# mgp25/OpenLTE

Measured on AMD Instinct MI355X. Metric: DL subframes/sec @20MHz 100RB 64QAM, full chain FFT->CE->demap->rate-unmatch->turbo(REF)->CRC (SURVEY 8d W4), higher is better.
Workload: dtype i8 IQ in, f32 FFT/CE/equaliser, i8 soft bits, i16 path metrics (differences exact modulo 2^16); 1 GPU; W4 full DL chain: 20 MHz/100 RB/64QAM, 9 allocations per subframe (8x12 PRB TBS 3240 + 1x4 PRB TBS 1064), 65536 subframes per GPU, int8 IQ in HBM; subframes_per_gpu=65536, N_ant=1, CFI=2, channel_estimate_form=compact, decoder=REF (reference-faithful, bit-exact), unique_subframes=96, streams_per_gpu=1

## Files before the change

openlte_amd/csrc/turbo.hip:

```cpp
#include <algorithm>
#include <cstring>
#include <initializer_list>
#include <type_traits>
#include <vector>

#include "plan_core.hpp"
#include "turbo_swar.h"

using namespace turbo_geom;

namespace {

constexpr uint32_t RX_NULL_AS_INT = 10000;


__device__ __forceinline__ int sbyte(uint32_t w, int k) { return (int)__builtin_amdgcn_sbfe(w, 8 * k, 8); }

typedef __attribute__((address_space(3))) const uint8_t  lds_u8_t;
typedef __attribute__((address_space(3))) const int8_t   lds_i8_t;
typedef __attribute__((address_space(3))) const uint16_t lds_u16_t;
__device__ __forceinline__ uint32_t lds_u8(uint32_t addr) { return *(lds_u8_t *)(uintptr_t)addr; }
__device__ __forceinline__ int      lds_i8(uint32_t addr) { return *(lds_i8_t *)(uintptr_t)addr; }
__device__ __forceinline__ uint32_t lds_u16(uint32_t addr) { return *(lds_u16_t *)(uintptr_t)addr; }

// ... 593 lines not shown
            uint32_t o[4];
#pragma unroll
            for (int j = 0; j < 4; j++)
                o[j] = pack4u(lds_u8(PREP_QTAB_AT + QTAB_HALF + v[Src::kPacked ? 0 : x][4 * j]), lds_u8(PREP_QTAB_AT + QTAB_HALF + v[Src::kPacked ? 0 : x][4 * j + 1]), lds_u8(PREP_QTAB_AT + QTAB_HALF + v[Src::kPacked ? 0 : x][4 * j + 2]), lds_u8(PREP_QTAB_AT + QTAB_HALF + v[Src::kPacked ? 0 : x][4 * j + 3]));
            Q[x] = make_uint4(o[0], o[1], o[2], o[3]);
        } else {
            int q[16];
            if (use_qtab) {
#pragma unroll
                for (int k = 0; k < 16; k++) {
                    const float f = v[Src::kPacked ? 0 : x][k];
                    const int   t = qtab[(int)fabsf(f)];
                    q[k]          = f < 0.0f ? -t : t;
                }
            } else {
#pragma unroll
                for (int k = 0; k < 16; k++) q[k] = (int)((float)v[Src::kPacked ? 0 : x][k] * 127.0f / mx);
            }
            Q[x] = pack16(q);
        }
        if (nv >= 0) *reinterpret_cast<uint4 *>(out.arr[x] + unit_off(tile_off, lane, u)) = Q[x];
    }
    if (nv >= 0) *reinterpret_cast<uint4 *>(q0_lds + 16 * u) = Q[0];
    __syncthreads();

    uint4 I0 = make_uint4(0, 0, 0, 0);
    if (nv > 0) {
        uint32_t idx[16];
        if constexpr (MULTI)
            load_idx16_at(reinterpret_cast<const_u32x4_t *>(reinterpret_cast<uintptr_t>(pi + 16 * (size_t)u)), nv, idx, K);
        else
            load_idx16(pi, u, nv, idx, K);
        I0 = gather16_bytes(PREP_Q0_AT, idx);
    }
    if (nv >= 0) *reinterpret_cast<uint4 *>(out.arr[3] + unit_off(tile_off, lane, u)) = I0;
    if (identity && src.hard_inputs()) {
        auto cnt4 = [](uint32_t a, uint32_t b) { return (a & 0x01010101u) + (b & 0x01010101u); };
        const uint32_t c1[4] = {cnt4(Q[1].x, Q[0].x), cnt4(Q[1].y, Q[0].y), cnt4(Q[1].z, Q[0].z), cnt4(Q[1].w, Q[0].w)};
        const uint32_t c2[4] = {cnt4(Q[2].x, I0.x), cnt4(Q[2].y, I0.y), cnt4(Q[2].z, I0.z), cnt4(Q[2].w, I0.w)};
        const uint32_t o1 = c1[0] | c1[1] | c1[2] | c1[3], o2 = c2[0] | c2[1] | c2[2] | c2[3];
        int w1max = (o1 & 0x02020202u) ? 254 : (o1 ? 127 : 0), w2max = (o2 & 0x02020202u) ? 254 : (o2 ? 127 : 0);
        block_max_i2(w1max, w2max, red_i);
        if (w1max != 0 && w2max != 0) {
            auto mag4 = [](uint32_t cnt, int W) { return W == 254 ? (cnt << 6) - ((cnt | (cnt >> 1)) & 0x01010101u) : (cnt << 7) - cnt; };
            if (nv >= 0) {
                *reinterpret_cast<uint4 *>(out.arr[4] + unit_off(tile_off, lane, u)) = make_uint4(mag4(c1[0], w1max), mag4(c1[1], w1max), mag4(c1[2], w1max), mag4(c1[3], w1max));
                *reinterpret_cast<uint4 *>(out.arr[5] + unit_off(tile_off, lane, u)) = make_uint4(mag4(c2[0], w2max), mag4(c2[1], w2max), mag4(c2[2], w2max), mag4(c2[3], w2max));
            }
            return;
        }
    }
    uint32_t w1[16], w2[16], w1m = 0, w2m = 0;
    abs_sum16(Q[1], Q[0], w1, w1m);
    abs_sum16(Q[2], I0, w2, w2m);
    int w1max = (int)w1m, w2max = (int)w2m;
    block_max_i2(w1max, w2max, red_i);
    auto closed = [](int W) { return W == 254 || W == 127; };
    auto closed16 = [](const uint32_t (&w)[16], int W) {
        uint32_t o[4];
#pragma unroll
        for (int j = 0; j < 4; j++) {
            const uint32_t p = pack4u(w[4 * j], w[4 * j + 1], w[4 * j + 2], w[4 * j + 3]);
            o[j] = W == 254 ? (p >> 1) & 0x7F7F7F7Fu : p;
        }
        return make_uint4(o[0], o[1], o[2], o[3]);
    };
    if (!(closed(w1max) && closed(w2max))) {
        const float W1 = (float)w1max, W2 = (float)w2max;
        for (uint32_t t = threadIdx.x; t < MTAB_N; t += blockDim.x) {
            const float w = (float)t;
            mtab1[t] = (int8_t)(int)(127.0f * (w / W1));
            mtab2[t] = (int8_t)(int)(127.0f * (w / W2));
        }
        __syncthreads();
    }
    if (nv >= 0) {
        *reinterpret_cast<uint4 *>(out.arr[4] + unit_off(tile_off, lane, u)) = closed(w1max) ? closed16(w1, w1max) : lookup16(0, w1);
        *reinterpret_cast<uint4 *>(out.arr[5] + unit_off(tile_off, lane, u)) = closed(w2max) ? closed16(w2, w2max) : lookup16(MTAB_N, w2);
    }
}


struct SisoPass {
    const uint8_t *in_a;
    const uint8_t *in_b;
    uint32_t      *sgn;
    uint32_t      *dec;
};
struct SisoArgs { SisoPass p[2]; };

typedef unsigned short v2u __attribute__((ext_vector_type(2)));
__device__ __forceinline__ uint32_t sign_bits(v2s n) { return __builtin_bit_cast(uint32_t, __builtin_bit_cast(v2u, n) >> 15); }

template <int S> __device__ __forceinline__ void acs_step2(v2s (&pm)[8], v2s x2, v2s y2, uint32_t &acc)
{
    const v2s mx = as_v2s(neg_mask(x2 ^ y2)), nmx = ~mx;
    const v2s uP = (x2 + y2) & nmx;
    const v2s uQ = (x2 - y2) & mx;
    const uint32_t m0p = neg_mask(x2) & 0xFFF8FFF8u;
    const v2s P2 = as_v2s(__builtin_amdgcn_bitop3_b32(as_u32(mx), m0p, 0xFFFCFFFCu, 0x06));
    const v2s Q2 = as_v2s(__builtin_amdgcn_bitop3_b32(as_u32(mx), m0p, 0xFFFCFFFCu, 0x60));
    const v2s n0 = pm[1] - pm[0], n1 = pm[3] - pm[2], n2 = pm[5] - pm[4], n3 = pm[7] - pm[6];
    constexpr uint32_t top = 0x00010001u << (15 - 4 * S);
    acc = __builtin_amdgcn_bitop3_b32(acc, neg_mask(n0), top, 0xF8);
    acc = __builtin_amdgcn_bitop3_b32(acc, neg_mask(n1), top >> 1, 0xF8);
    acc = __builtin_amdgcn_bitop3_b32(acc, neg_mask(n2), top >> 2, 0xF8);
    acc = __builtin_amdgcn_bitop3_b32(acc, neg_mask(n3), top >> 3, 0xF8);
    auto sel = [](v2s d, v2s yes, v2s no) { return bit_select(neg_mask(d), yes, no); };
    v2s nw[8];
    nw[0] = sel(n0 - P2, pm[1] + uP, pm[0] - uP);
    nw[4] = sel(n0 + P2, pm[1] - uP, pm[0] + uP);
    nw[1] = sel(n1 - Q2, pm[3] + uQ, pm[2] - uQ);
    nw[5] = sel(n1 + Q2, pm[3] - uQ, pm[2] + uQ);
    nw[2] = sel(n2 + Q2, pm[5] - uQ, pm[4] + uQ);
    nw[6] = sel(n2 - Q2, pm[5] + uQ, pm[4] - uQ);
    nw[3] = sel(n3 + P2, pm[7] - uP, pm[6] + uP);
    nw[7] = sel(n3 - P2, pm[7] + uP, pm[6] - uP);
#pragma unroll
    for (int s = 0; s < 8; s++) pm[s] = nw[s];
}

template <int R> __device__ __forceinline__ v2s byte_pair2(uint32_t w0, uint32_t w1)
{
    return as_v2s(__builtin_amdgcn_perm(w1, w0, (uint32_t)(4 + R) << 24 | 0x0C0000u | (uint32_t)R << 8 | 0x0Cu)) >> 7;
}


#ifndef SISO_WPE
#define SISO_WPE 4
#endif
template <bool MULTI, int MODE>
__global__ __launch_bounds__(256) __attribute__((amdgpu_waves_per_eu(SISO_WPE, 8))) void k_turbo_siso(SisoArgs args, uint32_t K_arg, uint32_t n_tiles_arg, MultiArgs ma,
                                                                                                         const uint32_t *__restrict__ order)
{
    constexpr uint32_t mode = MODE;
    constexpr int      NA = MODE ? 1 : 2;
    __shared__ uint32_t tb_lut[2048];
    for (uint32_t i = threadIdx.x; i < 2048; i += blockDim.x) tb_lut[i] = turbo_swar::traceback_entry(i >> 3, i & 7u);
    __syncthreads();
    const uint32_t lane = threadIdx.x & 63u;
    uint32_t       K = K_arg, n_tiles = n_tiles_arg, wv = blockIdx.x * 4 + (threadIdx.x >> 6), n_wv = mode ? n_tiles : (n_tiles + 1) / 2;
    size_t         seg_off = 0;
    if constexpr (MULTI) {
        if (order) wv = __builtin_amdgcn_readfirstlane(order[wv]);
        if (wv >= n_tiles_arg) return;
        const_seg_t &sg = multi_seg(ma, wv);
        K = sg.K; n_tiles = sg.n_tiles; seg_off = sg.arr_off;
        wv -= mode ? sg.wv23 : sg.wv1;
        n_wv = mode ? n_tiles : (n_tiles + 1) / 2;
    }
    const uint32_t Kp = kpad64(K), nblk = Kp >> 6;
    if (wv >= n_wv) return;
    const uint8_t *pa[2], *pb[2];
    uint32_t      *dec[2], *sgn[2];
#pragma unroll
    for (int h = 0; h < 2; h++) {
        const SisoPass &ps   = args.p[mode ? h : 0];
        const uint32_t  tile = mode ? wv : min(2 * wv + h, n_tiles - 1);
        const size_t    off  = seg_off + (size_t)tile * Kp * 64 + lane * 64;
        pa[h] = ps.in_a + off; pb[h] = ps.in_b + off;
        dec[h] = ps.dec + (seg_off >> 3) + ((size_t)tile * nblk * 64 + lane) * 8;
        sgn[h] = ps.sgn + (seg_off >> 5) + ((size_t)tile * nblk * 64 + lane) * 2;
    }

    v2s pm[8];
#pragma unroll
    for (int s = 0; s < 8; s++) pm[s] = (v2s)(0);

    uint4 A[NA][4], B[2][4];
#pragma unroll
    for (int h = 0; h < 2; h++)
#pragma unroll
        for (int q = 0; q < 4; q++) {
            if (h < NA) A[h][q] = reinterpret_cast<const uint4 *>(pa[h])[q];
            B[h][q] = reinterpret_cast<const uint4 *>(pb[h])[q];
        }
    for (uint32_t blk = 0; blk < nblk; blk++) {
        const uint32_t nxt = (blk + 1 < nblk) ? blk + 1 : blk;
        uint32_t       dw[2][8];
#pragma unroll
        for (int q = 0; q < 4; q++) {
#pragma unroll
            for (int g2 = 0; g2 < 2; g2++) {
                const int g = 2 * q + g2;
                uint32_t  acc_lo = 0, acc_hi = 0;
                if (blk * 64 + g * 8 < K) {
                    const uint32_t a0l = g2 ? A[0][q].z : A[0][q].x, a0h = g2 ? A[0][q].w : A[0][q].y;
                    const uint32_t a1l = g2 ? A[NA - 1][q].z : A[NA - 1][q].x, a1h = g2 ? A[NA - 1][q].w : A[NA - 1][q].y;
                    const uint32_t b0l = g2 ? B[0][q].z : B[0][q].x, b0h = g2 ? B[0][q].w : B[0][q].y;
                    const uint32_t b1l = g2 ? B[1][q].z : B[1][q].x, b1h = g2 ? B[1][q].w : B[1][q].y;
                    acs_step2<0>(pm, byte_pair2<0>(a0l, a1l), byte_pair2<0>(b0l, b1l), acc_lo);
                    acs_step2<1>(pm, byte_pair2<1>(a0l, a1l), byte_pair2<1>(b0l, b1l), acc_lo);
                    acs_step2<2>(pm, byte_pair2<2>(a0l, a1l), byte_pair2<2>(b0l, b1l), acc_lo);
                    acs_step2<3>(pm, byte_pair2<3>(a0l, a1l), byte_pair2<3>(b0l, b1l), acc_lo);
                    acs_step2<0>(pm, byte_pair2<0>(a0h, a1h), byte_pair2<0>(b0h, b1h), acc_hi);
                    acs_step2<1>(pm, byte_pair2<1>(a0h, a1h), byte_pair2<1>(b0h, b1h), acc_hi);
                    acs_step2<2>(pm, byte_pair2<2>(a0h, a1h), byte_pair2<2>(b0h, b1h), acc_hi);
                    acs_step2<3>(pm, byte_pair2<3>(a0h, a1h), byte_pair2<3>(b0h, b1h), acc_hi);
                }
                dw[0][g] = __builtin_amdgcn_perm(acc_lo, acc_hi, 0x05040100u);
                dw[1][g] = __builtin_amdgcn_perm(acc_lo, acc_hi, 0x07060302u);
            }
            if (q >= 2) {
#pragma unroll
                for (int qq = (q == 2 ? 0 : 3); qq <= (q == 2 ? 2 : 3); qq++)
#pragma unroll
                    for (int h = 0; h < 2; h++) {
                        if (h < NA) A[h][qq] = reinterpret_cast<const uint4 *>(pa[h] + (size_t)nxt * 4096)[qq];
                        B[h][qq] = reinterpret_cast<const uint4 *>(pb[h] + (size_t)nxt * 4096)[qq];
                    }
            }
        }
#pragma unroll
        for (int h = 0; h < 2; h++) {
            uint4 *dp = reinterpret_cast<uint4 *>(dec[h] + (size_t)blk * 64 * 8);
            dp[0] = make_uint4(dw[h][0], dw[h][1], dw[h][2], dw[h][3]);
            dp[1] = make_uint4(dw[h][4], dw[h][5], dw[h][6], dw[h][7]);
        }
    }

    int cur[2] = {0, 0};
    {
        int best[2] = {0, 0};
#pragma unroll
        for (int s = 1; s < 8; s++) {
            const uint32_t d  = as_u32(pm[s] - pm[0]);
            const int      dh[2] = {(int)__builtin_amdgcn_sbfe(d, 0, 16), (int)d >> 16};
#pragma unroll
            for (int h = 0; h < 2; h++)
                if (dh[h] < best[h]) { best[h] = dh[h]; cur[h] = s; }
        }
    }

    uint4 D[2][2], Dn[2][2];
#pragma unroll
    for (int h = 0; h < 2; h++) {
        const uint4 *dp = reinterpret_cast<const uint4 *>(dec[h] + (size_t)(nblk - 1) * 64 * 8);
        D[h][0] = dp[0];
        D[h][1] = dp[1];
    }
    for (int blk = (int)nblk - 1; blk >= 0; blk--) {
        const int prv = blk > 0 ? blk - 1 : 0;
#pragma unroll
        for (int h = 0; h < 2; h++) {
            const uint4 *dpn = reinterpret_cast<const uint4 *>(dec[h] + (size_t)prv * 64 * 8);
            Dn[h][0] = dpn[0];
            Dn[h][1] = dpn[1];
        }
        uint32_t sbits[2][2];
#pragma unroll
        for (int g = 7; g >= 0; g--) {
            if ((g & 3) == 3) sbits[0][g >> 2] = sbits[1][g >> 2] = 0;
            if ((uint32_t)blk * 64 + g * 8 < K) {
                uint32_t word[2];
#pragma unroll
                for (int h = 0; h < 2; h++) {
                    const uint4 dq = D[h][g >> 2];
                    word[h] = (g & 3) == 0 ? dq.x : (g & 3) == 1 ? dq.y : (g & 3) == 2 ? dq.z : dq.w;
                }
#pragma unroll
                for (int b = 0; b < 4; b++) {
#pragma unroll
                    for (int h = 0; h < 2; h++) {
                        const uint32_t e = tb_lut[((word[h] >> (8 * b)) & 0xFFu) << 3 | (uint32_t)cur[h]];
                        cur[h]           = (int)(e & 7u);
                        sbits[h][g >> 2]   = __builtin_amdgcn_alignbit(sbits[h][g >> 2], e, 30);
                    }
                }
            }
        }
#pragma unroll
        for (int h = 0; h < 2; h++) {
            *reinterpret_cast<uint2 *>(sgn[h] + (size_t)blk * 64 * 2) = make_uint2(sbits[h][0], sbits[h][1]);
            D[h][0] = Dn[h][0];
            D[h][1] = Dn[h][1];
        }
    }
}

struct SmallPar { uint32_t cw, uw; };

__device__ __forceinline__ uint2 map_compose(uint2 F, uint2 G)
{
    return make_uint2(__builtin_amdgcn_perm(F.y, F.x, G.x), __builtin_amdgcn_perm(F.y, F.x, G.y));
}
__device__ __forceinline__ uint32_t map_at(uint2 F, uint32_t s) { return ((s & 4u ? F.y : F.x) >> (8 * (s & 3u))) & 7u; }
template <int N> __device__ __forceinline__ uint2 map_row_shl(uint2 v, uint2 keep)
{
    return make_uint2((uint32_t)__builtin_amdgcn_update_dpp((int)keep.x, (int)v.x, 0x100 + N, 0xF, 0xF, false),
                      (uint32_t)__builtin_amdgcn_update_dpp((int)keep.y, (int)v.y, 0x100 + N, 0xF, 0xF, false));
}

template <bool MULTI>
__global__ __launch_bounds__(64) void k_turbo_siso_small(SisoArgs args, uint32_t K_arg, uint32_t n_cb_arg, uint32_t mode, uint32_t gpw, MultiArgs ma)
{
    extern __shared__ __attribute__((aligned(16))) uint32_t sm_small[];
    SmallPar (*par)[64][4] = reinterpret_cast<SmallPar(*)[64][4]>(sm_small);
    uint32_t K = K_arg, n_cb = n_cb_arg, bidx = blockIdx.x;
    size_t   seg_off = 0;
    if constexpr (MULTI) {
        const_seg_t &sg = multi_seg(ma, blockIdx.x);
        K = sg.K; n_cb = sg.n_cb; seg_off = sg.arr_off; bidx = blockIdx.x - (mode ? sg.ws23 : sg.ws1);
    }
    const uint32_t Kp = kpad64(K), n_w32 = Kp >> 5;
    uint32_t      *decw = sm_small + gpw * 64 * 4 * 2;
    const uint32_t lane = threadIdx.x, gi = lane >> 2, j = lane & 3u;
    const uint32_t T0 = bidx * gpw, n_tr = n_cb * (mode ? 2u : 1u);
    const uint32_t n_g = min(gpw, n_tr - T0);
    auto pass_of = [&](uint32_t g) -> const SisoPass & { return args.p[mode ? (T0 + g) & 1u : 0u]; };
    auto off_of  = [&](uint32_t g) -> size_t {
        const uint32_t cb = mode ? (T0 + g) >> 1 : T0 + g;
        return seg_off + (size_t)(cb >> 6) * Kp * 64 + (cb & 63u) * 64;
    };
    const uint32_t n_chunk = (K + 63) >> 6;

    uint32_t XY = 0;
    uint32_t accv = 0;
    const uint32_t half_sel = j < 2 ? 0x01000100u : 0x03020302u;
#ifdef SMALL_PAD
    uint32_t padv[4] = {lane, lane + 1, lane + 2, lane + 3};
#endif
    int xs[SMALL_G], ys[SMALL_G];
    auto fetch = [&](uint32_t ch) {
#pragma unroll
        for (uint32_t g = 0; g < SMALL_G; g++)
            if (g < n_g) {
                const size_t e = off_of(g) + (size_t)ch * 4096 + lane;
                xs[g] = (int8_t)pass_of(g).in_a[e];
                ys[g] = (int8_t)pass_of(g).in_b[e];
            }
    };
    fetch(0);
    for (uint32_t ch = 0; ch < n_chunk; ch++) {
#pragma unroll
        for (uint32_t g = 0; g < SMALL_G; g++) {
            if (g >= n_g) break;
            const int      x  = xs[g], y = ys[g];
            const int      m0 = x >> 31, mx = m0 ^ (y >> 31), nmx = ~mx;
            const int      uP = ((x + y) << 1) & nmx, uQ = ((x - y) << 1) & mx;
            const int      c4 = (m0 & 8) - 4, P2 = c4 & nmx, Q2 = c4 & mx;
            auto pm16 = [](int v) { return ((uint32_t)v & 0xFFFFu) | ((uint32_t)(-v) << 16); };
            const uint32_t cP = pm16(P2), uPw = pm16(uP), cQ = pm16(Q2), uQw = pm16(uQ);
            auto swp = [](uint32_t w) { return (w >> 16) | (w << 16); };
            uint4 *dst = reinterpret_cast<uint4 *>(&par[g][lane][0]);
            dst[0] = make_uint4(cP, uPw, cQ, uQw);
            dst[1] = make_uint4(swp(cQ), swp(uQw), swp(cP), swp(uPw));
        }
        __syncthreads();
        if (ch + 1 < n_chunk) fetch(ch + 1);
        const uint32_t n_t = min(64u, K - ch * 64);
        if (gi < n_g) {
            auto steps8 = [&](uint32_t t8) {
                SmallPar pr[8];
#pragma unroll
                for (int k = 0; k < 8; k++) pr[k] = par[gi][t8 + k][j];
#pragma unroll
                for (int k = 0; k < 8; k++) {
                    const uint32_t t0 = (uint32_t)__builtin_amdgcn_mov_dpp((int)XY, 0x88, 0xF, 0xF, false);
                    const uint32_t t1 = (uint32_t)__builtin_amdgcn_mov_dpp((int)XY, 0xDD, 0xF, 0xF, false);
                    const v2s a = as_v2s(__builtin_amdgcn_perm(t0, t0, half_sel)), b = as_v2s(__builtin_amdgcn_perm(t1, t1, half_sel));
                    const v2s n = b - a;
                    accv = __builtin_amdgcn_alignbit(accv, as_u32(n), 31);
                    const v2s uw = as_v2s(pr[k].uw);
                    XY = as_u32(bit_select(neg_mask(n - as_v2s(pr[k].cw)), b + uw, a - uw));
#ifdef SMALL_PAD
#pragma unroll
                    for (int z = 0; z < SMALL_PAD; z++) asm volatile("v_add_u32 %0, %0, %1" : "+v"(padv[z & 3]) : "v"(lane));
#endif
                }
            };
            uint32_t t = 0;
            for (; t + 32 <= n_t; t += 32) {
                steps8(t); steps8(t + 8); steps8(t + 16); steps8(t + 24);
                decw[(gi * n_w32 + ((ch * 64 + t) >> 5)) * 4 + j] = accv;
            }
            if (t < n_t) {
                const uint32_t w = (ch * 64 + t) >> 5, left = n_t - t;
                for (; t < n_t; t += 8) steps8(t);
                decw[(gi * n_w32 + w) * 4 + j] = accv << (32u - left);
            }
        }
        __syncthreads();
    }

#ifdef SMALL_PAD
    if ((padv[0] ^ padv[1] ^ padv[2] ^ padv[3]) == 0x12345678u) decw[0] = 0;
#endif
    uint32_t cur = 0;
    {
        const uint32_t q0 = (uint32_t)__builtin_amdgcn_mov_dpp((int)XY, 0x00, 0xF, 0xF, false), q1 = (uint32_t)__builtin_amdgcn_mov_dpp((int)XY, 0x55, 0xF, 0xF, false);
        const uint32_t q2 = (uint32_t)__builtin_amdgcn_mov_dpp((int)XY, 0xAA, 0xF, 0xF, false), q3 = (uint32_t)__builtin_amdgcn_mov_dpp((int)XY, 0xFF, 0xF, 0xF, false);
        const short pm[8] = {(short)q0, (short)q1, (short)q2, (short)q3, (short)(q0 >> 16), (short)(q1 >> 16), (short)(q2 >> 16), (short)(q3 >> 16)};
        int best = 0;
#pragma unroll
        for (int st = 1; st < 8; st++) {
            const int d = (short)(pm[st] - pm[0]);
            if (d < best) { best = d; cur = st; }
        }
    }

    const uint2 MAP_ID = make_uint2(0x03020100u, 0x07060504u);
    for (uint32_t g = 0; g < n_g; g++) {
        uint32_t       end = (uint32_t)__builtin_amdgcn_readlane((int)cur, (int)(g * 4));
        const uint32_t cb  = mode ? (T0 + g) >> 1 : T0 + g;
        uint32_t      *sgn = pass_of(g).sgn + (seg_off >> 5) + ((size_t)(cb >> 6) * n_chunk * 64 + (cb & 63u)) * 2;
        for (int ch = (int)n_chunk - 1; ch >= 0; ch--) {
            const uint32_t t = (uint32_t)ch * 64 + lane;
            const uint4    w = *reinterpret_cast<const uint4 *>(&decw[(g * n_w32 + (t >> 5)) * 4]);
            const uint32_t sh = 31u - (t & 31u);
            uint2          G = MAP_ID;
            if (t < K) {
                const uint32_t f = 0x06040200u + (((w.x >> sh) & 1u) | ((w.y >> sh) & 1u) << 8 | ((w.z >> sh) & 1u) << 16 | ((w.w >> sh) & 1u) << 24);
                G = make_uint2(f, f);
            }
            G = map_compose(G, map_row_shl<1>(G, MAP_ID));
            G = map_compose(G, map_row_shl<2>(G, MAP_ID));
            G = map_compose(G, map_row_shl<4>(G, MAP_ID));
            G = map_compose(G, map_row_shl<8>(G, MAP_ID));
            const uint32_t row = lane >> 4;
#pragma unroll
            for (int r = 1; r < 4; r++) {
                const uint2 R = make_uint2((uint32_t)__builtin_amdgcn_readlane((int)G.x, 16 * r), (uint32_t)__builtin_amdgcn_readlane((int)G.y, 16 * r));
                if (row < (uint32_t)r) G = map_compose(G, R);
            }
            const uint2    Gn  = make_uint2((uint32_t)__shfl_down((int)G.x, 1u), (uint32_t)__shfl_down((int)G.y, 1u));
            const uint32_t nxt = lane == 63 ? end : map_at(Gn, end);
            const uint32_t st  = map_at(G, end);
            const bool     pos = (nxt < st) || (nxt == st && nxt == 0);
            const uint64_t neg = __ballot(t < K && !pos);
            if (lane == 0) *reinterpret_cast<uint2 *>(sgn + (size_t)ch * 64 * 2) = make_uint2((uint32_t)neg, (uint32_t)(neg >> 32));
            end = (uint32_t)__builtin_amdgcn_readlane((int)st, 0);
        }
    }
}

namespace sw = turbo_swar;
struct UnitWords { uint32_t w[5]; };
__device__ __forceinline__ UnitWords load_unit_words(const uint8_t *arr, size_t tile_off, uint32_t lane, uint32_t u)
{
    const uint4 c    = *reinterpret_cast<const uint4 *>(arr + unit_off(tile_off, lane, u));
    uint32_t    prev = 0x7F7F7F7Fu;
    if (u > 0) prev = *reinterpret_cast<const uint32_t *>(arr + unit_off(tile_off, lane, u - 1) + 12);
    return UnitWords{{prev, c.x, c.y, c.z, c.w}};
}
__device__ __forceinline__ UnitWords load_unit_joined(const uint8_t *mag, const uint32_t *sgn, size_t tile_off, uint32_t lane, uint32_t u)
{
    UnitWords      w = load_unit_words(mag, tile_off, lane, u);
    const uint32_t *sp = sgn + (tile_off >> 5) + ((size_t)(u >> 2) * 64 + lane) * 2;
    const uint2    c = *reinterpret_cast<const uint2 *>(sp);
    uint32_t       ph = 0;
    if ((u & 3u) == 0 && u > 0) ph = sp[1 - 128];
    const uint32_t b = sw::unit_sign_bits(c.x, c.y, ph, u);
    if (u > 0) w.w[0] = sw::joined_from_bits(w.w[0], b & 15u);
#pragma unroll
    for (int j = 0; j < 4; j++) w.w[j + 1] = sw::joined_from_bits(w.w[j + 1], (b >> (4 * j + 4)) & 15u);
    return w;
}
struct PermArgs { const uint8_t *M1; const uint32_t *S1;  const uint8_t *X2; uint8_t *out[2];  };

#ifndef PERM_NB
#define PERM_NB 4
#endif
static_assert(PERM_NB == PERM_BLOCKS, "a size's perm grid is a multiple of 128 workgroups (the merged decode's map granularity) only for four blocks per workgroup");
template <int NSLOT, bool MULTI = false>
__global__ __launch_bounds__(384) void k_turbo_perm(PermArgs a, uint32_t K_arg, uint32_t n_cb_arg, const uint16_t *__restrict__ pi_arg, MultiArgs ma)
{
    static_assert(NSLOT == 1, "one unit per thread");
    uint32_t K = K_arg, n_cb = n_cb_arg, bidx = blockIdx.x, grid = gridDim.x;
    size_t   seg_off = 0;
    const uint16_t *__restrict__ pi = pi_arg;
    if constexpr (MULTI) {
        const_seg_t &sg = multi_seg(ma, blockIdx.x >> 7);
        K = sg.K; n_cb = sg.n_cb; pi = (const uint16_t *)sg.pi; bidx = blockIdx.x - sg.wg_perm; grid = sg.perm_grid;
        seg_off = sg.arr_off;
    }
    extern __shared__ __attribute__((aligned(16))) int8_t smp[];
    int8_t *mtab = smp, *sm = smp + MTAB_N;
    const uint32_t Kp = kpad64(K), n_units = Kp >> 4;
    int           *red_i = reinterpret_cast<int *>(sm + Kp);
    const uint32_t u0 = threadIdx.x;
    const int      nv = (u0 < n_units) ? min(16, max(0, (int)K - 16 * (int)u0)) : -1;
    IdxRaw         praw;
    {
        const uint4 *ip = reinterpret_cast<const uint4 *>(pi + 16 * (size_t)(nv > 0 ? u0 : 0));
        const uint32_t kk = K | K << 16;
        praw.lo = ip[0];
        praw.hi = (nv > 8) ? ip[1] : make_uint4(kk, kk, kk, kk);
    }
#pragma unroll 1
    for (uint32_t it = 0; it < PERM_NB; it++) {
        const uint32_t cb = xcd_cb(bidx + it * grid, n_cb), tile = cb >> 6, lane = cb & 63;
        const size_t   tile_off = seg_off + (size_t)tile * Kp * 64;
        if (cb >= n_cb) {
            if (MULTI && cb < ((n_cb + 63u) & ~63u) && nv >= 0) {
                *reinterpret_cast<uint4 *>(a.out[0] + unit_off(tile_off, lane, u0)) = make_uint4(0, 0, 0, 0);
                *reinterpret_cast<uint4 *>(a.out[1] + unit_off(tile_off, lane, u0)) = make_uint4(0, 0, 0, 0);
            }
            continue;
        }
        uint32_t u = u0;
        asm volatile("" : "+v"(u), "+v"(praw.lo.x), "+v"(praw.lo.y), "+v"(praw.lo.z), "+v"(praw.lo.w), "+v"(praw.hi.x), "+v"(praw.hi.y), "+v"(praw.hi.z), "+v"(praw.hi.w));
        uint4          X2 = make_uint4(0, 0, 0, 0);
        if (nv >= 0) {
            const UnitWords wa = load_unit_joined(a.M1, a.S1, tile_off, lane, u);
            uint32_t        pa = wa.w[0];
            X2 = *reinterpret_cast<const uint4 *>(a.X2 + unit_off(tile_off, lane, u));
            uint32_t c1[4];
#pragma unroll
            for (int j = 0; j < 4; j++) {
                const uint32_t ja = wa.w[j + 1];
                const sw::SM4  A  = sw::unjoin(ja);
                c1[j] = (4 * j < nv) ? sw::to_tc(sw::step3(A, sw::feedback(ja, pa))) : 0u;
                pa    = ja;
            }
            *reinterpret_cast<uint4 *>(sm + 16 * u) = make_uint4(c1[0], c1[1], c1[2], c1[3]);
        }
        __syncthreads();
        uint4 I1 = make_uint4(0, 0, 0, 0);
        if (nv > 0) {
            uint32_t idx[16];
            unpack_idx16(praw, idx);
            I1 = gather16_bytes(MTAB_N, idx);
        }
        if (nv >= 0) *reinterpret_cast<uint4 *>(a.out[0] + unit_off(tile_off, lane, u)) = I1;
        uint32_t w[16], wm = 0;
        if (nv <= 0) X2 = make_uint4(0, 0, 0, 0);
        abs_sum16(X2, I1, w, wm);
        const int   wmax = block_max_i((int)wm, red_i);
        if (wmax == 254 || wmax == 127) {
            uint32_t o[4];
#pragma unroll
            for (int j = 0; j < 4; j++) {
                const uint32_t p = pack4u(w[4 * j], w[4 * j + 1], w[4 * j + 2], w[4 * j + 3]);
                o[j] = wmax == 254 ? (p >> 1) & 0x7F7F7F7Fu : p;
            }
            if (nv >= 0) *reinterpret_cast<uint4 *>(a.out[1] + unit_off(tile_off, lane, u)) = make_uint4(o[0], o[1], o[2], o[3]);
            continue;
        }
        const float W = (float)wmax;
        for (uint32_t t = threadIdx.x; t < MTAB_N; t += blockDim.x) mtab[t] = (int8_t)(int)(127.0f * ((float)t / W));
        __syncthreads();
        if (nv >= 0) *reinterpret_cast<uint4 *>(a.out[1] + unit_off(tile_off, lane, u)) = lookup16(0, w);
        __syncthreads();
    }
}

struct VoteArgs { const uint8_t *X0, *M1, *M2, *M3; const uint32_t *S1, *S2, *S3; };

template <bool GROUP, int NSLOT, bool MULTI = false>
__global__ __launch_bounds__(384) __attribute__((amdgpu_waves_per_eu(6, 8))) void k_turbo_vote(VoteArgs a, uint32_t K_arg, uint32_t n_cb_arg, const uint16_t *__restrict__ inv_arg,
                                                    uint8_t *__restrict__ c_bits, GroupDesc g, MultiArgs ma)
{
    static_assert(NSLOT == 1, "one unit per thread");
    uint32_t K = K_arg, n_cb = n_cb_arg, bidx = blockIdx.x;
    size_t   seg_off = 0;
    const uint16_t *__restrict__ inv = inv_arg;
    if constexpr (MULTI) {
        const_seg_t &sg = multi_seg(ma, blockIdx.x >> 9);
        K = sg.K; n_cb = sg.n_cb; inv = (const uint16_t *)sg.inv2; bidx = blockIdx.x - sg.wg_cb; seg_off = sg.arr_off;
        g.desc += sg.cb_base;
    }
    extern __shared__ __attribute__((aligned(16))) int8_t sm[];
    const uint32_t cb = xcd_cb(bidx, n_cb), tile = cb >> 6, lane = cb & 63, Kp = kpad64(K), n_units = Kp >> 4;
    if (cb >= n_cb) return;
    const size_t   tile_off = seg_off + (size_t)tile * Kp * 64;
    int8_t        *d12 = sm, *bits = sm + 2 * Kp + 32;
    uint32_t      *red_u = reinterpret_cast<uint32_t *>(bits + Kp);
    const uint32_t u  = threadIdx.x;
    const int      nv = (u < n_units) ? min(16, max(0, (int)K - 16 * (int)u)) : -1;
    IdxRaw vraw;
    {
        const uint4 *ip = reinterpret_cast<const uint4 *>(inv + 16 * (size_t)(nv > 0 ? u : 0));
        vraw.lo = ip[0];
        vraw.hi = ip[1];
    }
    const uint32_t crc_w0 = (GROUP && nv > 0) ? g.crc_tab[MI_CRC_TAB_BIAS + K - 16 * u - 16] : 0u;
    v2s            s0e[4], s0o[4];
    if (threadIdx.x == 0) *reinterpret_cast<uint32_t *>(d12 + 2 * Kp) = 0u;
    if (nv >= 0) {
        const UnitWords wa = load_unit_joined(a.M1, a.S1, tile_off, lane, u), wb = load_unit_joined(a.M2, a.S2, tile_off, lane, u),
                        wc = load_unit_joined(a.M3, a.S3, tile_off, lane, u);
        uint32_t        pa = wa.w[0], pb = wb.w[0], pc = wc.w[0];
        const uint4    x0 = *reinterpret_cast<const uint4 *>(a.X0 + unit_off(tile_off, lane, u));
        const uint32_t x0w[4] = {x0.x, x0.y, x0.z, x0.w};
        uint32_t       dn[8];
#pragma unroll
        for (int j = 0; j < 4; j++) {
            const uint32_t ja = wa.w[j + 1], jb = wb.w[j + 1], jc = wc.w[j + 1];
            const sw::SM4  A = sw::unjoin(ja), B = sw::unjoin(jb), B_ = sw::unjoin(jc);
            const sw::SM4  F  = sw::feedback(ja, pa);
            const sw::SM4  G  = sw::feedback(jb, pb);
            const sw::SM4  G_ = sw::feedback(jc, pc);
            pa = ja; pb = jb; pc = jc;
            const uint32_t u1 = sw::step10_biased(A, B, G), n2 = sw::step11_neg_biased(B_, G_);
            const uint32_t de = sw::sub_halves(sw::even_halves(u1), sw::even_halves(n2)), dd = sw::sub_halves(sw::odd_halves(u1), sw::odd_halves(n2));
            const uint32_t x0b = x0w[j] ^ sw::HI, nc = sw::step3_neg_biased(A, F);
            s0e[j] = as_v2s(sw::sub_halves(sw::even_halves(x0b), sw::even_halves(nc)));
            s0o[j] = as_v2s(sw::sub_halves(sw::odd_halves(x0b), sw::odd_halves(nc)));
            const bool in = 4 * j < nv;
            dn[2 * j]     = in ? __builtin_amdgcn_perm(dd, de, 0x05040100u) : 0u;
            dn[2 * j + 1] = in ? __builtin_amdgcn_perm(dd, de, 0x07060302u) : 0u;
        }
        uint4 *dst = reinterpret_cast<uint4 *>(d12 + 32 * u);
        dst[0] = make_uint4(dn[0], dn[1], dn[2], dn[3]);
        dst[1] = make_uint4(dn[4], dn[5], dn[6], dn[7]);
    } else {
#pragma unroll
        for (int j = 0; j < 4; j++) s0e[j] = s0o[j] = (v2s)(0);
    }
    __syncthreads();
    uint32_t alloc = 0, tbs = 0, F = 0, crc = 0;
    if (GROUP) {
        alloc = g.desc[cb].alloc;
        tbs   = g.desc[cb].tbs;
        F     = K - tbs - 24;
    }
    if (nv > 0) {
        const uint32_t  iw[8] = {vraw.lo.x, vraw.lo.y, vraw.lo.z, vraw.lo.w, vraw.hi.x, vraw.hi.y, vraw.hi.z, vraw.hi.w};
        uint32_t        me[4], mo[4], bw[4];
#pragma unroll
        for (int j = 0; j < 4; j++) {
            const uint32_t i0 = iw[2 * j] & 0xFFFFu, i1 = iw[2 * j] >> 16, i2 = iw[2 * j + 1] & 0xFFFFu, i3 = iw[2 * j + 1] >> 16;
            const uint32_t ge = lds_u16(i0) | lds_u16(i2) << 16, go = lds_u16(i1) | lds_u16(i3) << 16;
            me[j] = as_u32((s0e[j] + as_v2s(ge)) >> 15);
            mo[j] = as_u32((s0o[j] + as_v2s(go)) >> 15);
            bw[j] = (me[j] & 0x00010001u) | (mo[j] & 0x00010001u) << 8;
        }
        if (GROUP) {
            if (!(nv == 16 && 16 * u >= F)) {
#pragma unroll
                for (int j = 0; j < 4; j++) {
                    auto ok = [&](int k) { return (k < nv && 16 * u + k >= F) ? 0xFFFFu : 0u; };
                    me[j] &= ok(4 * j) | ok(4 * j + 2) << 16;
                    mo[j] &= ok(4 * j + 1) | ok(4 * j + 3) << 16;
                }
            }
            const uint32_t GS = 0x864CFBu << 8;
            uint32_t       w = crc_w0;
#pragma unroll
            for (int k = 15; k >= 0; k--) {
                const int      j = k >> 2;
                const uint32_t m = (k & 3) == 0 ? (uint32_t)__builtin_amdgcn_sbfe(me[j], 0, 1) : (k & 3) == 1 ? (uint32_t)__builtin_amdgcn_sbfe(mo[j], 0, 1)
                                 : (k & 3) == 2 ? (uint32_t)((int)me[j] >> 31) : (uint32_t)((int)mo[j] >> 31);
                crc ^= w & m;
                if (k > 0) w = (w << 1) ^ ((uint32_t)((int)w >> 31) & GS);
            }
        }
        const uint4 pk = make_uint4(bw[0], bw[1], bw[2], bw[3]);
        if (GROUP) *reinterpret_cast<uint4 *>(bits + 16 * u) = pk;
        else {
            uint2 *o = reinterpret_cast<uint2 *>(c_bits + (size_t)cb * K + 16 * u);
            o[0] = make_uint2(pk.x, pk.y);
            if (nv > 8) o[1] = make_uint2(pk.z, pk.w);
        }
    }
    if (GROUP) {
        crc = wave_xor_u(crc);
        __syncthreads();
        if ((threadIdx.x & 63) == 0) red_u[threadIdx.x >> 6] = crc;
        __syncthreads();
        crc = 0;
        for (uint32_t w = 0; w < (blockDim.x >> 6); w++) crc ^= red_u[w];
        if (threadIdx.x == 0) g.status[alloc] = (crc == 0) ? 0  : 2 ;
        uint8_t *o = g.out_bits + (size_t)alloc * g.out_stride;
        if (g.packed && ((F | tbs) & 7u) == 0) {
            const uint32_t nby = tbs >> 3, nw = nby >> 2;
            auto byte_at = [&](uint32_t m) -> uint32_t {
                const uint2 w = *reinterpret_cast<const uint2 *>(bits + F + 8 * m);
                return (((w.x * 0x08040201u) >> 24) & 0xFu) << 4 | (((w.y * 0x08040201u) >> 24) & 0xFu);
            };
            for (uint32_t m = threadIdx.x; m < nw; m += blockDim.x)
                reinterpret_cast<uint32_t *>(o)[m] = byte_at(4 * m) | byte_at(4 * m + 1) << 8 | byte_at(4 * m + 2) << 16 | byte_at(4 * m + 3) << 24;
            for (uint32_t m = 4 * nw + threadIdx.x; m < nby; m += blockDim.x) o[m] = (uint8_t)byte_at(m);
        } else if (g.packed) {
            for (uint32_t m = threadIdx.x; m < (tbs + 7) >> 3; m += blockDim.x) {
                uint32_t v = 0;
                for (uint32_t b = 0; b < 8; b++) v = v << 1 | ((8 * m + b < tbs) ? ((uint32_t)bits[F + 8 * m + b] & 1u) : 0u);
                o[m] = (uint8_t)v;
            }
        } else if ((F & 3u) == 0) {
            const uint32_t nq = tbs >> 2;
            const uint32_t *bw = reinterpret_cast<const uint32_t *>(bits + F);
            for (uint32_t m = threadIdx.x; m < nq; m += blockDim.x) reinterpret_cast<uint32_t *>(o)[m] = bw[m];
            for (uint32_t m = 4 * nq + threadIdx.x; m < tbs; m += blockDim.x) o[m] = (uint8_t)bits[m + F];
        } else
            for (uint32_t m = threadIdx.x; m < tbs; m += blockDim.x) o[m] = (uint8_t)bits[m + F];
    }
}

__global__ __launch_bounds__(256) void k_cb_desc(GroupDesc g, uint32_t n_cb, const uint32_t *__restrict__ nnn, CbDesc *__restrict__ out)
{
    const uint32_t cb = blockIdx.x * blockDim.x + threadIdx.x;
    if (cb >= n_cb) return;
    const uint32_t a = g.cb_alloc[cb], txm = g.allocs[a].tx_mode;
    const uint32_t combo = g.ul ? 8u + (g.allocs[a].rv_idx & 3u)
                                : ((g.allocs[a].rv_idx & 3u) << 1) | ((txm == 3 || txm == 4 || txm == 8 || txm == 9) ? 1u : 0u);
    CbDesc d;
    d.alloc = a; d.e_off = g.e_off[a]; d.E = g.e_len[a]; d.combo = combo; d.Nnn = nnn[combo];
    d.hard  = (g.allocs[a].mod_type >= 2 && d.E <= d.Nnn) ? 1u : 0u;
    d.tbs   = g.allocs[a].tbs; d.pad = 0;
    out[cb] = d;
}

__global__ __launch_bounds__(256) void k_cb_desc_multi(GroupDesc g, uint32_t n_cb, const KSeg *__restrict__ segs, uint32_t n_seg, CbDesc *__restrict__ out)
{
    const uint32_t cb = blockIdx.x * blockDim.x + threadIdx.x;
    if (cb >= n_cb) return;
    uint32_t lo = 0, hi = n_seg;
    while (hi - lo > 1) {
        const uint32_t mid = (lo + hi) >> 1;
        if (segs[mid].cb_base <= cb) lo = mid; else hi = mid;
    }
    const uint32_t a = g.cb_alloc[cb], txm = g.allocs[a].tx_mode;
    const uint32_t combo = g.ul ? 8u + (g.allocs[a].rv_idx & 3u)
                                : ((g.allocs[a].rv_idx & 3u) << 1) | ((txm == 3 || txm == 4 || txm == 8 || txm == 9) ? 1u : 0u);
    CbDesc d;
    d.alloc = a; d.e_off = g.e_off[a]; d.E = g.e_len[a]; d.combo = combo; d.Nnn = segs[lo].nnn[combo];
    d.hard  = (g.allocs[a].mod_type >= 2 && d.E <= d.Nnn) ? 1u : 0u;
    d.tbs   = g.allocs[a].tbs; d.pad = 0;
    out[cb] = d;
}

__global__ __launch_bounds__(256) void k_rm_rank_table(uint32_t K, uint16_t *__restrict__ tabs, uint32_t *__restrict__ nnn)
{
    const uint32_t combo = blockIdx.y, t = blockIdx.x * blockDim.x + threadIdx.x;
    RmGeom rm;
    if (combo < 8) rm.init(K + 4, (combo & 1) ? 3 : 1, combo >> 1);
    else           rm.init(K + 4, 1, combo - 8, 1, 1, 1, false);
    if (t == 0) nnn[combo] = rm.Nnn;
    if (t >= 3 * K) return;
    const uint32_t x = t / K, i = t - x * K;
    uint32_t p, c;
    rm.pos_cnt(i, (int)x, p, c);
    uint32_t k = 0xFFFFu;
    if (p < rm.N_cb) k = (p >= rm.k0m) ? c - rm.cnt_k0 : rm.Nnn - rm.cnt_k0 + c;
    tabs[(size_t)combo * 3 * K + t] = (uint16_t)k;
}

struct RmParams { uint32_t D, E, C, tx_mode, N_soft, M_dl_harq, limited, rv; };

__global__ __launch_bounds__(256) void k_rate_unmatch_f32(const float *__restrict__ e, RmParams pr, uint32_t n_cb,
                                                          float *__restrict__ d)
// ... 538 lines not shown
```

openlte_amd/csrc/turbo_swar.h:

```cpp
#pragma once

#include <cstdint>

#ifdef __HIPCC__
#define SWAR_FN __host__ __device__ __forceinline__
#else
#define SWAR_FN inline
#endif

namespace turbo_swar {

constexpr uint32_t HI = 0x80808080u, LO7 = 0x7F7F7F7Fu, ONES = 0x01010101u, EVEN = 0x00FF00FFu;

SWAR_FN uint32_t alignbit(uint32_t hi, uint32_t lo, uint32_t sh)
{
#if defined(__HIP_DEVICE_COMPILE__)
    return __builtin_amdgcn_alignbit(hi, lo, sh);
#else
    return (uint32_t)((((uint64_t)hi << 32) | lo) >> sh);
#endif
}
SWAR_FN uint32_t sub_halves(uint32_t a, uint32_t b)
{
#if defined(__HIP_DEVICE_COMPILE__)
    typedef short v2s_t __attribute__((ext_vector_type(2)));
    return __builtin_bit_cast(uint32_t, __builtin_bit_cast(v2s_t, a) - __builtin_bit_cast(v2s_t, b));
#else
    return ((a - (b & 0xFFFFu)) & 0xFFFFu) | ((a & 0xFFFF0000u) - (b & 0xFFFF0000u));
#endif
}

struct SM4 { uint32_t m, s; };

SWAR_FN uint32_t low7(uint32_t bits) { return bits - (bits >> 7); }

SWAR_FN uint32_t to_joined(uint32_t w)
{
    const uint32_t s = w & HI, t = s >> 7;
    return (w ^ (s - t)) + t;
}
SWAR_FN uint32_t joined_from(uint32_t m, uint32_t neg_mask) { return m | (neg_mask & (m + LO7) & HI); }
SWAR_FN uint32_t joined_from_bits(uint32_t m, uint32_t nib) { return m | ((nib * 0x10204080u) & (m + LO7) & HI); }
SWAR_FN uint32_t unit_sign_bits(uint32_t c_lo, uint32_t c_hi, uint32_t prev_hi, uint32_t u)
{
    const uint32_t q = u & 3u;
    const uint64_t c = ((uint64_t)c_hi << 32) | c_lo;
    return q ? (uint32_t)(c >> (16u * q - 4u)) & 0xFFFFFu : (c_lo & 0xFFFFu) << 4 | prev_hi >> 28;
}
SWAR_FN SM4 unjoin(uint32_t j) { return SM4{j & LO7, j & HI}; }
SWAR_FN SM4 split(uint32_t w) { return unjoin(to_joined(w)); }
SWAR_FN uint32_t join(const SM4 &a) { return a.m | a.s; }
SWAR_FN uint32_t to_tc(const SM4 &a)
{
    const uint32_t t = a.s >> 7;
    return ((a.m ^ (a.s - t)) + t) | a.s;
}

SWAR_FN uint32_t biased(uint32_t x, uint32_t neg)
{
    const uint32_t t = neg >> 7;
    return ((x ^ (neg - t)) + t) + (neg ^ HI);
}
SWAR_FN uint32_t even_halves(uint32_t w) { return w & EVEN; }
SWAR_FN uint32_t odd_halves(uint32_t w) { return (w >> 8) & EVEN; }

SWAR_FN uint32_t half_sum(uint32_t ma, uint32_t mb) { return ((ma + mb) >> 1) & LO7; }
SWAR_FN SM4 soft_xor(const SM4 &a, const SM4 &b)
{
    const uint32_t m = half_sum(a.m, b.m);
    return SM4{m, (a.s ^ b.s) & (m + LO7) & HI};
}

SWAR_FN uint32_t delay2(uint32_t cur, uint32_t prev) { return alignbit(cur, prev, 16); }
SWAR_FN uint32_t delay3(uint32_t cur, uint32_t prev) { return alignbit(cur, prev, 8); }
SWAR_FN SM4 feedback(uint32_t cur_joined, uint32_t prev_joined)
{
    const uint32_t d2 = delay2(cur_joined, prev_joined), d3 = delay3(cur_joined, prev_joined);
    const uint32_t x = d2 ^ d3;
    const uint32_t m = (d2 & d3 & LO7) + ((x >> 1) & 0x3F3F3F3Fu);
    return SM4{m, x & (m + LO7) & HI};
}

SWAR_FN SM4 step3(const SM4 &A, const SM4 &F) { return soft_xor(A, F); }
SWAR_FN uint32_t step3_neg_biased(const SM4 &A, const SM4 &F) { return biased(half_sum(A.m, F.m), A.s ^ F.s ^ HI); }

SWAR_FN uint32_t avg_biased(uint32_t xb, uint32_t yb) { return (xb & yb) + (((xb ^ yb) >> 1) & LO7); }

SWAR_FN uint32_t step10_biased(const SM4 &A, const SM4 &B, const SM4 &G)
{
    const uint32_t mx = B.s ^ G.s, tm = mx >> 7, m7 = mx - tm;
    const uint32_t y  = (A.m & m7) | (B.m & ~m7);
    const uint32_t w  = avg_biased(G.m | HI, biased(y, mx & (A.s ^ B.s)));
    return (w ^ (m7 | mx)) + tm;
}
SWAR_FN uint32_t step11_neg_biased(const SM4 &B, const SM4 &G)
{
    const uint32_t mx = B.s ^ G.s, tm = mx >> 7, m7 = mx - tm;
    const uint32_t w  = avg_biased(B.m | HI, biased(G.m, mx & B.s));
    return (w ^ ~(m7 | mx)) + (tm ^ ONES);
}

SWAR_FN uint32_t traceback_entry(uint32_t byte, uint32_t cur)
{
    uint32_t sgn = 0;
    for (int k = 0; k < 2; k++) {
        const uint32_t nib = k ? byte >> 4 : byte & 15u;
        const uint32_t j = cur & 3u, bit = (nib >> (3 - j)) & 1u, st = 2 * j + bit;
        const bool     pos = (cur < st) || (cur == st && cur == 0);
        if (!pos) sgn |= k ? 1u << 30 : 1u << 31;
        cur = st;
    }
    return cur | sgn;
}

}
```

Before: 2.838 million subframes/s.

## Transpose sign-bit planes to per-lane contiguous layout with staged vector stores

Changes the traceback sign-bit storage from a tile-interleaved layout (one uint2 per lane per block, lanes strided) to a per-lane contiguous layout with a bit-plane permutation inside each 32-bit word, so consumers extract unit signs with shifts instead of 64-bit funnel extraction. The traceback kernel stages four blocks of sign words in registers and emits 16-byte vector stores, while the parallel traceback path shuffles bits into the new plane order before ballot. Consumers (permute and SISO input loaders) are rewritten to decode signs directly from one word plus a halo. It also makes tile bases wave-uniform via readfirstlane. The aim is fewer scattered small stores and cheaper sign unpacking, at the cost of extra register staging, per-lane select logic and a shuffle in the ballot path.

```diff
diff --git a/openlte_amd/csrc/turbo.hip b/openlte_amd/csrc/turbo.hip
--- a/openlte_amd/csrc/turbo.hip
+++ b/openlte_amd/csrc/turbo.hip
@@ -769,15 +769,15 @@
     const uint32_t Kp = kpad64(K), nblk = Kp >> 6;
     if (wv >= n_wv) return;
     const uint8_t *pa[2], *pb[2];
-    uint32_t      *dec[2], *sgn[2];
+    uint32_t      *dec[2];
+    const uint32_t dec_at = lane * 8;
 #pragma unroll
     for (int h = 0; h < 2; h++) {
         const SisoPass &ps   = args.p[mode ? h : 0];
         const uint32_t  tile = mode ? wv : min(2 * wv + h, n_tiles - 1);
         const size_t    off  = seg_off + (size_t)tile * Kp * 64 + lane * 64;
         pa[h] = ps.in_a + off; pb[h] = ps.in_b + off;
-        dec[h] = ps.dec + (seg_off >> 3) + ((size_t)tile * nblk * 64 + lane) * 8;
-        sgn[h] = ps.sgn + (seg_off >> 5) + ((size_t)tile * nblk * 64 + lane) * 2;
+        dec[h] = ps.dec + (seg_off >> 3) + (size_t)__builtin_amdgcn_readfirstlane(tile) * nblk * 64 * 8;
     }
 
     v2s pm[8];
@@ -830,7 +830,7 @@
         }
 #pragma unroll
         for (int h = 0; h < 2; h++) {
-            uint4 *dp = reinterpret_cast<uint4 *>(dec[h] + (size_t)blk * 64 * 8);
+            uint4 *dp = reinterpret_cast<uint4 *>(dec[h] + (dec_at + blk * 64 * 8));
             dp[0] = make_uint4(dw[h][0], dw[h][1], dw[h][2], dw[h][3]);
             dp[1] = make_uint4(dw[h][4], dw[h][5], dw[h][6], dw[h][7]);
         }
@@ -849,10 +849,16 @@
         }
     }
 
-    uint4 D[2][2], Dn[2][2];
+    typedef uint32_t sign4_t __attribute__((ext_vector_type(4), aligned(8)));
+    uint32_t  stg[2][8] = {};
+    uint4     D[2][2], Dn[2][2];
+    uint32_t      *sgn[2];
+    const uint32_t sgn_at = (uint32_t)turbo_swar::sign_word_index(lane, nblk, 0);
 #pragma unroll
     for (int h = 0; h < 2; h++) {
-        const uint4 *dp = reinterpret_cast<const uint4 *>(dec[h] + (size_t)(nblk - 1) * 64 * 8);
+        const uint32_t tile = __builtin_amdgcn_readfirstlane(mode ? wv : min(2 * wv + h, n_tiles - 1));
+        sgn[h] = args.p[mode ? h : 0].sgn + (seg_off >> 5) + (size_t)tile * nblk * 64 * 2;
+        const uint4 *dp = reinterpret_cast<const uint4 *>(dec[h] + (dec_at + (nblk - 1) * 64 * 8));
         D[h][0] = dp[0];
         D[h][1] = dp[1];
     }
@@ -860,14 +866,15 @@
         const int prv = blk > 0 ? blk - 1 : 0;
 #pragma unroll
         for (int h = 0; h < 2; h++) {
-            const uint4 *dpn = reinterpret_cast<const uint4 *>(dec[h] + (size_t)prv * 64 * 8);
+            const uint4 *dpn = reinterpret_cast<const uint4 *>(dec[h] + (dec_at + (uint32_t)prv * 64 * 8));
             Dn[h][0] = dpn[0];
             Dn[h][1] = dpn[1];
         }
-        uint32_t sbits[2][2];
+        const uint32_t slot = (lane * nblk + (uint32_t)blk) & 3u;
+        uint32_t sacc[2][2];
 #pragma unroll
         for (int g = 7; g >= 0; g--) {
-            if ((g & 3) == 3) sbits[0][g >> 2] = sbits[1][g >> 2] = 0;
+            if ((g & 3) == 3) sacc[0][0] = sacc[0][1] = sacc[1][0] = sacc[1][1] = 0;
             if ((uint32_t)blk * 64 + g * 8 < K) {
                 uint32_t word[2];
 #pragma unroll
@@ -881,14 +888,35 @@
                     for (int h = 0; h < 2; h++) {
                         const uint32_t e = tb_lut[((word[h] >> (8 * b)) & 0xFFu) << 3 | (uint32_t)cur[h]];
                         cur[h]           = (int)(e & 7u);
-                        sbits[h][g >> 2]   = __builtin_amdgcn_alignbit(sbits[h][g >> 2], e, 30);
+                        sacc[h][b & 1]   = turbo_swar::sign_acc_push(sacc[h][b & 1], e);
                     }
                 }
             }
+            if ((g & 3) == 0) {
+#pragma unroll
+                for (int h = 0; h < 2; h++) {
+                    const uint32_t w = turbo_swar::sign_word_join(sacc[h][0], sacc[h][1]);
+#pragma unroll
+                    for (int k = 0; k < 4; k++) stg[h][2 * k + (g >> 2)] = slot == (uint32_t)k ? w : stg[h][2 * k + (g >> 2)];
+                }
+            }
+        }
+        if (slot == 0 || blk == 0) {
+#pragma unroll
+            for (int h = 0; h < 2; h++) {
+                uint32_t *sp = sgn[h] + (sgn_at + 2 * (uint32_t)blk);
+                if (slot == 0 && (uint32_t)blk + 4 <= nblk) {
+                    *reinterpret_cast<sign4_t *>(sp)     = sign4_t{stg[h][0], stg[h][1], stg[h][2], stg[h][3]};
+                    *reinterpret_cast<sign4_t *>(sp + 4) = sign4_t{stg[h][4], stg[h][5], stg[h][6], stg[h][7]};
+                } else {
+#pragma unroll
+                    for (int k = 0; k < 4; k++)
+                        if ((uint32_t)k >= slot && (uint32_t)blk + k - slot < nblk) *reinterpret_cast<uint2 *>(sp + 2 * k - 2 * slot) = make_uint2(stg[h][2 * k], stg[h][2 * k + 1]);
+                }
+            }
         }
 #pragma unroll
         for (int h = 0; h < 2; h++) {
-            *reinterpret_cast<uint2 *>(sgn[h] + (size_t)blk * 64 * 2) = make_uint2(sbits[h][0], sbits[h][1]);
             D[h][0] = Dn[h][0];
             D[h][1] = Dn[h][1];
         }
@@ -1020,7 +1048,7 @@
     for (uint32_t g = 0; g < n_g; g++) {
         uint32_t       end = (uint32_t)__builtin_amdgcn_readlane((int)cur, (int)(g * 4));
         const uint32_t cb  = mode ? (T0 + g) >> 1 : T0 + g;
-        uint32_t      *sgn = pass_of(g).sgn + (seg_off >> 5) + ((size_t)(cb >> 6) * n_chunk * 64 + (cb & 63u)) * 2;
+        uint32_t      *sgn = pass_of(g).sgn + (seg_off >> 5) + (size_t)(cb >> 6) * n_chunk * 64 * 2 + turbo_swar::sign_word_index(cb & 63u, n_chunk, 0);
         for (int ch = (int)n_chunk - 1; ch >= 0; ch--) {
             const uint32_t t = (uint32_t)ch * 64 + lane;
             const uint4    w = *reinterpret_cast<const uint4 *>(&decw[(g * n_w32 + (t >> 5)) * 4]);
@@ -1044,8 +1072,8 @@
             const uint32_t nxt = lane == 63 ? end : map_at(Gn, end);
             const uint32_t st  = map_at(G, end);
             const bool     pos = (nxt < st) || (nxt == st && nxt == 0);
-            const uint64_t neg = __ballot(t < K && !pos);
-            if (lane == 0) *reinterpret_cast<uint2 *>(sgn + (size_t)ch * 64 * 2) = make_uint2((uint32_t)neg, (uint32_t)(neg >> 32));
+            const uint64_t neg = __ballot(__shfl((int)(t < K && !pos), (int)turbo_swar::sign_plane_lane(lane)) != 0);
+            if (lane == 0) *reinterpret_cast<uint2 *>(sgn + 2 * ch) = make_uint2((uint32_t)neg, (uint32_t)(neg >> 32));
             end = (uint32_t)__builtin_amdgcn_readlane((int)st, 0);
         }
     }
@@ -1060,18 +1088,20 @@
     if (u > 0) prev = *reinterpret_cast<const uint32_t *>(arr + unit_off(tile_off, lane, u - 1) + 12);
     return UnitWords{{prev, c.x, c.y, c.z, c.w}};
 }
-__device__ __forceinline__ UnitWords load_unit_joined(const uint8_t *mag, const uint32_t *sgn, size_t tile_off, uint32_t lane, uint32_t u)
-{
-    UnitWords      w = load_unit_words(mag, tile_off, lane, u);
-    const uint32_t *sp = sgn + (tile_off >> 5) + ((size_t)(u >> 2) * 64 + lane) * 2;
-    const uint2    c = *reinterpret_cast<const uint2 *>(sp);
-    uint32_t       ph = 0;
-    if ((u & 3u) == 0 && u > 0) ph = sp[1 - 128];
-    const uint32_t b = sw::unit_sign_bits(c.x, c.y, ph, u);
-    if (u > 0) w.w[0] = sw::joined_from_bits(w.w[0], b & 15u);
-#pragma unroll
-    for (int j = 0; j < 4; j++) w.w[j + 1] = sw::joined_from_bits(w.w[j + 1], (b >> (4 * j + 4)) & 15u);
-    return w;
+struct UnitSigned {
+    uint32_t halo, m[4], x;
+    __device__ __forceinline__ sw::SM4 word(int j) const { return sw::SM4{m[j], sw::signed_under(m[j], x, j)}; }
+};
+__device__ __forceinline__ UnitSigned load_unit_signed(const uint8_t *mag, const uint32_t *sgn, size_t tile_off, uint32_t lane, uint32_t nblk, uint32_t u)
+{
+    const UnitWords w  = load_unit_words(mag, tile_off, lane, u);
+    const uint32_t *sp = sgn + (tile_off >> 5) + sw::sign_word_index(lane, nblk, u >> 1);
+    const uint32_t  S = sp[0];
+    uint32_t        Sb = 0;
+    if ((u & 1u) == 0 && u > 0) Sb = sp[-1];
+    UnitSigned r{w.w[0], {w.w[1], w.w[2], w.w[3], w.w[4]}, sw::sign_unit(S, u)};
+    if (u > 0) r.halo |= sw::signed_under_flags(r.halo, sw::sign_halo(S, Sb, u));
+    return r;
 }
 struct PermArgs { const uint8_t *M1; const uint32_t *S1;  const uint8_t *X2; uint8_t *out[2];  };
 
@@ -1119,14 +1149,14 @@
         asm volatile("" : "+v"(u), "+v"(praw.lo.x), "+v"(praw.lo.y), "+v"(praw.lo.z), "+v"(praw.lo.w), "+v"(praw.hi.x), "+v"(praw.hi.y), "+v"(praw.hi.z), "+v"(praw.hi.w));
         uint4          X2 = make_uint4(0, 0, 0, 0);
         if (nv >= 0) {
-            const UnitWords wa = load_unit_joined(a.M1, a.S1, tile_off, lane, u);
-            uint32_t        pa = wa.w[0];
+            const UnitSigned ua = load_unit_signed(a.M1, a.S1, tile_off, lane, n_units >> 2, u);
+            uint32_t         pa = ua.halo;
             X2 = *reinterpret_cast<const uint4 *>(a.X2 + unit_off(tile_off, lane, u));
             uint32_t c1[4];
 #pragma unroll
             for (int j = 0; j < 4; j++) {
-                const uint32_t ja = wa.w[j + 1];
-                const sw::SM4  A  = sw::unjoin(ja);
+                const sw::SM4  A  = ua.word(j);
+                const uint32_t ja = sw::join(A);
                 c1[j] = (4 * j < nv) ? sw::to_tc(sw::step3(A, sw::feedback(ja, pa))) : 0u;
                 pa    = ja;
             }
@@ -1195,16 +1225,16 @@
     v2s            s0e[4], s0o[4];
     if (threadIdx.x == 0) *reinterpret_cast<uint32_t *>(d12 + 2 * Kp) = 0u;
     if (nv >= 0) {
-        const UnitWords wa = load_unit_joined(a.M1, a.S1, tile_off, lane, u), wb = load_unit_joined(a.M2, a.S2, tile_off, lane, u),
-                        wc = load_unit_joined(a.M3, a.S3, tile_off, lane, u);
-        uint32_t        pa = wa.w[0], pb = wb.w[0], pc = wc.w[0];
+        const UnitSigned ua = load_unit_signed(a.M1, a.S1, tile_off, lane, n_units >> 2, u), ub = load_unit_signed(a.M2, a.S2, tile_off, lane, n_units >> 2, u),
+                         uc = load_unit_signed(a.M3, a.S3, tile_off, lane, n_units >> 2, u);
+        uint32_t        pa = ua.halo, pb = ub.halo, pc = uc.halo;
         const uint4    x0 = *reinterpret_cast<const uint4 *>(a.X0 + unit_off(tile_off, lane, u));
         const uint32_t x0w[4] = {x0.x, x0.y, x0.z, x0.w};
         uint32_t       dn[8];
 #pragma unroll
         for (int j = 0; j < 4; j++) {
-            const uint32_t ja = wa.w[j + 1], jb = wb.w[j + 1], jc = wc.w[j + 1];
-            const sw::SM4  A = sw::unjoin(ja), B = sw::unjoin(jb), B_ = sw::unjoin(jc);
+            const sw::SM4  A = ua.word(j), B = ub.word(j), B_ = uc.word(j);
+            const uint32_t ja = sw::join(A), jb = sw::join(B), jc = sw::join(B_);
             const sw::SM4  F  = sw::feedback(ja, pa);
             const sw::SM4  G  = sw::feedback(jb, pb);
             const sw::SM4  G_ = sw::feedback(jc, pc);
diff --git a/openlte_amd/csrc/turbo_swar.h b/openlte_amd/csrc/turbo_swar.h
--- a/openlte_amd/csrc/turbo_swar.h
+++ b/openlte_amd/csrc/turbo_swar.h
@@ -1,5 +1,6 @@
 #pragma once
 
+#include <cstddef>
 #include <cstdint>
 
 #ifdef __HIPCC__
@@ -40,12 +41,30 @@
     return (w ^ (s - t)) + t;
 }
 SWAR_FN uint32_t joined_from(uint32_t m, uint32_t neg_mask) { return m | (neg_mask & (m + LO7) & HI); }
-SWAR_FN uint32_t joined_from_bits(uint32_t m, uint32_t nib) { return m | ((nib * 0x10204080u) & (m + LO7) & HI); }
-SWAR_FN uint32_t unit_sign_bits(uint32_t c_lo, uint32_t c_hi, uint32_t prev_hi, uint32_t u)
+
+SWAR_FN uint32_t sign_plane_bit(uint32_t t) { return 8u * (t & 3u) + ((t >> 2) & 7u); }
+SWAR_FN uint32_t sign_plane_step(uint32_t p) { return 4u * (p & 7u) + ((p >> 3) & 3u); }
+SWAR_FN size_t   sign_word_index(uint32_t lane, uint32_t nblk, uint32_t word) { return (size_t)lane * 2u * nblk + word; }
+SWAR_FN uint32_t sign_flags(uint32_t S, uint32_t g) { return ((S >> (g & 7u)) & ONES) << 7; }
+SWAR_FN uint32_t sign_unit(uint32_t S, uint32_t u) { return S >> (4u * (u & 1u)); }
+SWAR_FN uint32_t signed_under_flags(uint32_t m, uint32_t flags) { return flags & (m + LO7) & HI; }
+SWAR_FN uint32_t signed_under(uint32_t m, uint32_t x, int j) { return signed_under_flags(m, x << (7 - j)); }
+SWAR_FN uint32_t sign_halo(uint32_t S, uint32_t S_before, uint32_t u) { return (u & 1u) ? S << 4 : S_before; }
+SWAR_FN uint32_t sign_acc_push(uint32_t acc, uint32_t entry) { return (acc << 1) | entry; }
+SWAR_FN uint32_t sign_word_join(uint32_t acc32, uint32_t acc10)
 {
-    const uint32_t q = u & 3u;
-    const uint64_t c = ((uint64_t)c_hi << 32) | c_lo;
-    return q ? (uint32_t)(c >> (16u * q - 4u)) & 0xFFFFFu : (c_lo & 0xFFFFu) << 4 | prev_hi >> 28;
+#if defined(__HIP_DEVICE_COMPILE__)
+    return __builtin_amdgcn_perm(acc32, acc10, 0x07060302u);
+#else
+    return (acc32 & 0xFFFF0000u) | (acc10 >> 16);
+#endif
+}
+SWAR_FN uint32_t sign_plane_lane(uint32_t L) { return (L & 32u) | sign_plane_step(L & 31u); }
+SWAR_FN uint32_t sign_word_from_steps(uint64_t steps, uint32_t h)
+{
+    uint32_t S = 0;
+    for (uint32_t p = 0; p < 32; p++) S |= (uint32_t)((steps >> sign_plane_lane(32u * h + p)) & 1u) << p;
+    return S;
 }
 SWAR_FN SM4 unjoin(uint32_t j) { return SM4{j & LO7, j & HI}; }
 SWAR_FN SM4 split(uint32_t w) { return unjoin(to_joined(w)); }
@@ -107,7 +126,7 @@
         const uint32_t nib = k ? byte >> 4 : byte & 15u;
         const uint32_t j = cur & 3u, bit = (nib >> (3 - j)) & 1u, st = 2 * j + bit;
         const bool     pos = (cur < st) || (cur == st && cur == 0);
-        if (!pos) sgn |= k ? 1u << 30 : 1u << 31;
+        if (!pos) sgn |= k ? 1u << 16 : 1u << 24;
         cur = st;
     }
     return cur | sgn;
```

After: 2.901 million subframes/s (median of 6 runs). 1.02x the previous value.
